# asharakeh/pod_compare

Hardware: AMD Instinct MI355X
Metric: images/sec (BayesOD+MC-dropout, 1280x720) (higher is better)
Workload: dtype f32 (convolutions: every fp32 product from 2-way f16 splits of the power-of-two-scaled fp32 operands, 3 partial products, fp32 accumulate; closer to fp64 than the fp32 MFMA: profiles/r05_f16_split_numerics.txt)

## Files before the change

### pod_compare_amd/csrc/k11_wino_conv.hip

```cpp
#include "pod_wino.h"

namespace pod {

__global__ void __launch_bounds__(256) k_wino_filter(const float* __restrict__ w, float* __restrict__ U, int32_t K, int32_t C, int32_t Kpad) {
    const int64_t t = (int64_t)blockIdx.x * blockDim.x + threadIdx.x;
    if (t >= (int64_t)Kpad * C) return;
    const int k = (int)(t / C), c = (int)(t % C);
    float u[4][6];
    wino_filter_values(w, k, c, K, C, u);
    const int nchunk = C / 8, ks = k >> 6, j64 = k & 63, ch = c >> 3, cc = c & 7;
    const int h = cc >> 2, sc = cc & 3;
    float* dst = U + ((int64_t)ks * nchunk + ch) * WINO_U_FLOATS + (h * 64 + j64) * 4 + sc;
#pragma unroll
    for (int q = 0; q < 24; ++q) dst[q * 512] = u[q / 6][q % 6];
}

__global__ void __launch_bounds__(256, 1) k_wino_conv3x3(const WinoParams P) {
    extern __shared__ __attribute__((aligned(16))) float lds[];
    const int tid = threadIdx.x, lane = tid & 63, wave = tid >> 6;
    int ks, tb;
    wino_schedule(P.KS, P.n_blocks, ks, tb);
    if (tb >= P.n_blocks) return;
    WINO_STAMP(0);
    WINO_STAMP_WALL(12);
// ... 125 lines not shown
    __builtin_amdgcn_s_waitcnt(WINO_WAIT_VM16);
    __builtin_amdgcn_s_barrier();
    WINO_STAMP(1);
    WINO_READ_MINI(0, 0); WINO_READ_MINI(0, 1); WINO_READ_MINI(0, 2); WINO_READ_MINI(0, 3); WINO_READ_MINI(0, 4); WINO_READ_MINI(0, 5);
    WINO_READ_MINI(0, 6); WINO_READ_MINI(0, 7); WINO_READ_MINI(0, 8); WINO_READ_MINI(0, 9); WINO_READ_MINI(0, 10); WINO_READ_MINI(0, 11);
    __builtin_amdgcn_s_waitcnt(WINO_WAIT_LGKM0);
    __builtin_amdgcn_sched_barrier(0);
#pragma unroll
    for (int i = 0; i < 10; ++i) transform_piece(vA, i);
    __builtin_amdgcn_sched_barrier(0);
    asm volatile("s_nop 1");
    WINO_STAMP(2);
    const f32x16 zero16 = {0.f, 0.f, 0.f, 0.f, 0.f, 0.f, 0.f, 0.f, 0.f, 0.f, 0.f, 0.f, 0.f, 0.f, 0.f, 0.f};
    auto chunk = [&](auto first, auto c_t, auto par_t, int sc, f32x4(&vC)[6], f32x4(&uC)[12], f32x4(&vN)[6], f32x4(&uN)[12]) {
        constexpr int c = decltype(c_t)::value, par = decltype(par_t)::value;
        constexpr int rc = (c + 1) & 3, rpar = c == 3 ? par ^ 1 : par;
        constexpr int ph = c == 3 ? 0 : c + 1, dpar = c == 3 ? par : par ^ 1;
        const int ch = 4 * sc + c, c1 = ch + 1 < nchunk ? ch + 1 : last;
        const int fs0 = c == 3 ? sc + 2 : sc + 1, fs = fs0 < last_s ? fs0 : last_s;
        float* wr = lds + dpar * WINO_SB_FLOATS;
        wino_static_for([&](auto J) __attribute__((always_inline)) {
            constexpr int j = decltype(J)::value;
            if constexpr (decltype(first)::value && j < 12) acc[j] = __builtin_amdgcn_mfma_f32_32x32x2f32(uC[j][0], vC[j >> 1][0], zero16, 0, 0, 0);
            else WINO_MFMA(vC, uC, j);
            if constexpr (j < 12) {
                if constexpr (decltype(first)::value) WINO_READ_MINI(1, j);
                else if (!(POD_WINO_ELIM & 1)) WINO_READ(rpar, rc, j);
            }
            else if constexpr (j < 24) { if (!(POD_WINO_ELIM & 2)) filter_piece(c1, uN, j - 12); }
            else if constexpr (j == 24) __builtin_amdgcn_s_waitcnt(WINO_WAIT_LGKM0);
            else if constexpr (j >= 25 && j < 35) { if (!(POD_WINO_ELIM & 8)) transform_piece(vN, j - 25); }
            else if constexpr (j >= 36 && j <= 45 && (j - 36) % 3 == 0 && c != 2) { if (!(POD_WINO_ELIM & 4)) wino_patch_piece(r_rsrc, wr, a, fs, 4 * ph + (j - 36) / 3, doff[4 * ph + (j - 36) / 3]); }
            __builtin_amdgcn_sched_barrier(0);
        }, std::make_integer_sequence<int, 48>{});
        if (!(POD_WINO_ELIM & 16)) {
            __builtin_amdgcn_s_waitcnt(c != 2 ? WINO_WAIT_VM4 : WINO_WAIT_VM0);
            __builtin_amdgcn_s_barrier();
        }
    };
    using std::integral_constant;
    chunk(std::true_type{}, integral_constant<int, 0>{}, integral_constant<int, 0>{}, 0, vA, uA, vB, uB);
    for (int base = 0;; base += 8) {
#define WINO_CHUNK(t)                                                                                                              \
    if (base + (t) >= nchunk) break;                                                                                               \
    if ((t) & 1) chunk(std::false_type{}, integral_constant<int, (t) & 3>{}, integral_constant<int, ((t) >> 2) & 1>{}, (base + (t)) >> 2, vB, uB, vA, uA); \
    else chunk(std::false_type{}, integral_constant<int, (t) & 3>{}, integral_constant<int, ((t) >> 2) & 1>{}, (base + (t)) >> 2, vA, uA, vB, uB);
        WINO_CHUNK(1) WINO_CHUNK(2) WINO_CHUNK(3) WINO_CHUNK(4) WINO_CHUNK(5) WINO_CHUNK(6) WINO_CHUNK(7) WINO_CHUNK(8)
#undef WINO_CHUNK
    }
#undef WINO_MFMA
    __syncthreads();
    WINO_STAMP(3);

    if (!wino_output_stage(acc, lds, a, i32, h)) return;
    const WinoStore S{P.sets.out[0], P.sets.bias[0], nullptr, 1.0f, P.sets.offset[0], 0, P.sets.k_planes[0]};
    if (S.k_planes > 0) wino_store_planes(P, B, S, lds, ks);
    else wino_store_channels_last(P, B, S, lds, ks);
    WINO_STAMP_END();
}

}

#ifdef POD_TRACE
extern "C" int pod_wino_trace_dump(long long* host, int32_t n_workgroups) { return pod::wino_trace_dump(host, n_workgroups); }
#endif

extern "C" int pod_wino_filter_transform(const float* weight, float* U, int32_t K, int32_t C, pod_stream_t stream) {
    if (!weight || !U || K < 1 || C < 8 || (C & 7) != 0) return POD_E_INVALID;
    const int32_t Kpad = (K + 63) / 64 * 64;
    const int64_t n = (int64_t)Kpad * C;
    hipLaunchKernelGGL(pod::k_wino_filter, dim3((unsigned)((n + 255) / 256)), dim3(256), 0, (hipStream_t)stream, weight, U, K, C, Kpad);
    POD_CHECK_LAUNCH();
    return POD_OK;
}

extern "C" int pod_wino_conv3x3(const float* in, float* out, const float* U, const float* bias, const int32_t* blocks, int32_t n_blocks,
                                int32_t C, int32_t K, int32_t k_planes, int32_t relu, float p, uint64_t seed, uint64_t offset,
                                const uint64_t* epoch, pod_stream_t stream) {
    if (!in || !out || in == out || !U || !blocks || n_blocks < 0 || C < 8 || (C & 7) != 0 || K < 64 || (K & 63) != 0 ||
        !(p >= 0.0f && p < 1.0f) || k_planes < 0 || k_planes > K || (k_planes > 0 && p != 0.0f))
        return POD_E_INVALID;
    pod::WinoParams P{};
    const int64_t grid = pod::wino_params_launch(P, blocks, n_blocks, C, K, relu, p, seed, epoch);
    if (grid < 0) return POD_E_INVALID;
    if (((reinterpret_cast<uintptr_t>(in) | reinterpret_cast<uintptr_t>(out) | reinterpret_cast<uintptr_t>(U) |
          reinterpret_cast<uintptr_t>(bias) | reinterpret_cast<uintptr_t>(blocks)) & 15u) != 0)
        return POD_E_INVALID;
    if (n_blocks == 0) return POD_OK;
    if (pod_lds_opt_in<pod::k_wino_conv3x3>(pod::WINO_LDS_BYTES) != POD_OK) return POD_E_LAUNCH;
    pod::wino_params_set(P, 0, 0, in, out, U, bias, nullptr, nullptr, offset, 0, k_planes);
    hipLaunchKernelGGL(pod::k_wino_conv3x3, dim3((unsigned)grid), dim3(256), pod::WINO_LDS_BYTES, (hipStream_t)stream, P);
    POD_CHECK_LAUNCH();
    return POD_OK;
}
```

### pod_compare_amd/csrc/k12_wino_conv_split.hip

```cpp
#include "pod_wino.h"

namespace pod {

typedef uint32_t vu32x4 __attribute__((ext_vector_type(4)));
constexpr int WINO_US_BYTES = 24 * 2 * 2 * 64 * 16;
constexpr int WINO_U_TOP = 14, WINO_V_TOP = 9;
constexpr int WINO_WAIT_VM24 = 0x4078;

__global__ void __launch_bounds__(256) k_wino_filter_amax(const float* __restrict__ w, float* __restrict__ amax, int32_t K, int32_t C, int32_t Kpad) {
    const int64_t t = (int64_t)blockIdx.x * blockDim.x + threadIdx.x;
    float m = 0.0f;
    if (t < (int64_t)Kpad * C) {
        float u[4][6];
        wino_filter_values(w, (int)(t / C), (int)(t % C), K, C, u);
#pragma unroll
        for (int i = 0; i < 24; ++i) m = fmaxf(m, fabsf(u[i / 6][i % 6]));
    }
    wino_publish_amax1(amax, m);
}
__global__ void __launch_bounds__(256) k_wino_filter_split(const float* __restrict__ w, uint16_t* __restrict__ Us, const float* __restrict__ amax,
                                                           int32_t K, int32_t C, int32_t Kpad) {
    const int64_t t = (int64_t)blockIdx.x * blockDim.x + threadIdx.x;
    if (t >= (int64_t)Kpad * C) return;
    const int k = (int)(t / C), c = (int)(t % C);
// ... 270 lines not shown
            if constexpr (mode == 0 && prod == 0)
                acc[p * 2 + kb] = __builtin_amdgcn_mfma_f32_32x32x16_f16(__builtin_bit_cast(wino_f16x8, uP[p][kb * 2 + sa]), __builtin_bit_cast(wino_f16x8, Vb[p][sb]), zero16, 0, 0, 0);
            else
                acc[p * 2 + kb] = __builtin_amdgcn_mfma_f32_32x32x16_f16(__builtin_bit_cast(wino_f16x8, uP[p][kb * 2 + sa]), __builtin_bit_cast(wino_f16x8, Vb[p][sb]), acc[p * 2 + kb], 0, 0, 0);
            if constexpr (m < 4) { if (!(POD_WINO_ELIM & 2)) filter_piece(p + WINO_U_LEAD >= 6 ? qn : q, (p + WINO_U_LEAD) % 6, uP[(p + WINO_U_LEAD) % 6], m); }
            else if constexpr (m == 4) { if (!(POD_WINO_ELIM & 4)) stage_write(c16 == 0 ? par ^ 1 : par, p, c16 == 0 ? 6 + p : p); }
            if constexpr (p == 5 && m >= 4) {
                if (!(POD_WINO_ELIM & 4)) {
                    stage_load(3 * (m - 4), ls, 6 * c16 + 3 * (m - 4));
                    stage_load(3 * (m - 4) + 1, ls, 6 * c16 + 3 * (m - 4) + 1);
                    stage_load(3 * (m - 4) + 2, ls, 6 * c16 + 3 * (m - 4) + 2);
                }
            }
            if constexpr (mode != 0) {
                constexpr int u0 = j * N_UNITS / N_SLOTS, u1 = (j + 1) * N_UNITS / N_SLOTS;
                wino_static_for([&](auto K) __attribute__((always_inline)) {
                    unit(std::integral_constant<int, u0 + decltype(K)::value>{}, std::integral_constant<int, npar>{}, std::integral_constant<int, n16>{},
                         std::integral_constant<bool, mode == 2>{});
                }, std::make_integer_sequence<int, u1 - u0>{});
            }
            __builtin_amdgcn_sched_barrier(0);
        }, std::make_integer_sequence<int, N_SLOTS>{});
        __builtin_amdgcn_s_waitcnt(WINO_WAIT_LGKM0);
        __builtin_amdgcn_s_barrier();
        if constexpr (mode == 0) {
            if (q >= last) return;
            if constexpr (!(POD_WINO_ELIM & 1)) WINO_READ12(WINO_READ, npar, n16, 0);
            WINO_READS_LANDED();
            __builtin_amdgcn_sched_barrier(0);
            make_v(0);
            __builtin_amdgcn_sched_barrier(0);
            if constexpr (!(POD_WINO_ELIM & 1)) WINO_READ12(WINO_READ, npar, n16, 1);
            WINO_READS_LANDED();
            __builtin_amdgcn_sched_barrier(0);
            make_v(1);
            split_all();
            __builtin_amdgcn_sched_barrier(0);
            __builtin_amdgcn_s_barrier();
        }
    };
    using std::integral_constant;
    chunk(integral_constant<int, 0>{}, integral_constant<int, 0>{}, integral_constant<int, 0>{}, 0);
    if (nchunk > 1) chunk(integral_constant<int, 1>{}, integral_constant<int, 1>{}, integral_constant<int, 0>{}, 1);
    for (int base = 0;; base += 4) {
#define WINO_CHUNK(t)                                                                                                              \
    if (base + (t) >= nchunk) break;                                                                                               \
    chunk(integral_constant<int, 2>{}, integral_constant<int, (t) & 1>{}, integral_constant<int, ((t) >> 1) & 1>{}, base + (t));
        WINO_CHUNK(2) WINO_CHUNK(3) WINO_CHUNK(4) WINO_CHUNK(5)
#undef WINO_CHUNK
    }
    __syncthreads();
    WINO_STAMP(3);

    if (!wino_output_stage(acc, lds, a, i32, h)) return;
    const float inv = wino_pow2_inverse(sv) * wino_pow2_inverse(wino_pow2_scale(u_amax, WINO_U_TOP));
    const WinoStore S{set_out + (int64_t)blockIdx.y * P.split_out_stride, set_bias, set_out_amax, inv, set_offset, set_replicas, set_k_planes};
    const float lmax = S.k_planes > 0 ? wino_store_planes(P, B, S, lds, ks) : wino_store_channels_last(P, B, S, lds, ks);
    if (set_out_amax) wino_publish_amax_block(set_out_amax, lmax);
    WINO_STAMP_END();
}

}

#ifdef POD_TRACE
extern "C" int pod_wino_trace_dump_split(long long* host, int32_t n_workgroups) { return pod::wino_trace_dump(host, n_workgroups); }
#endif

extern "C" int64_t pod_wino_filter_split_bytes(int32_t K, int32_t C) {
    if (K < 1 || C < 16 || (C & 15) != 0) return 0;
    const int64_t Kpad = (K + 63) / 64 * 64;
    return Kpad / 64 * (C / 16) * (int64_t)pod::WINO_US_BYTES + 16;
}

extern "C" int pod_wino_filter_transform_split(const float* weight, void* Us, int32_t K, int32_t C, pod_stream_t stream) {
    if (!weight || !Us || K < 1 || C < 16 || (C & 15) != 0 || (reinterpret_cast<uintptr_t>(Us) & 15u) != 0) return POD_E_INVALID;
    const int32_t Kpad = (K + 63) / 64 * 64;
    const int64_t n = (int64_t)Kpad * C;
    float* amax = reinterpret_cast<float*>(reinterpret_cast<char*>(Us) + pod_wino_filter_split_bytes(K, C) - 16);
    if (hipMemsetAsync(amax, 0, 16, (hipStream_t)stream) != hipSuccess) return POD_E_LAUNCH;
    hipLaunchKernelGGL(pod::k_wino_filter_amax, dim3((unsigned)((n + 255) / 256)), dim3(256), 0, (hipStream_t)stream, weight, amax, K, C, Kpad);
    POD_CHECK_LAUNCH();
    hipLaunchKernelGGL(pod::k_wino_filter_split, dim3((unsigned)((n + 255) / 256)), dim3(256), 0, (hipStream_t)stream, weight,
                       reinterpret_cast<uint16_t*>(Us), amax, K, C, Kpad);
    POD_CHECK_LAUNCH();
    return POD_OK;
}

extern "C" int pod_wino_conv3x3_split(const PodWinoConv* d, pod_stream_t stream) {
    if (!d || d->n_sets < 1 || d->n_sets > 4 || !d->blocks || d->n_blocks < 0 || d->C < 16 || (d->C & 15) != 0 || d->K < 64 || (d->K & 63) != 0 ||
        !(d->p >= 0.0f && d->p < 1.0f) || d->sets[0].first_block != 0 || (reinterpret_cast<uintptr_t>(d->blocks) & 15u) != 0 ||
        d->reserved != 0)
        return POD_E_INVALID;
    const int32_t C = d->C, K = d->K;
    pod::WinoParams P{};
    const int64_t grid = pod::wino_params_launch(P, d->blocks, d->n_blocks, C, K, d->relu, d->p, d->seed, d->epoch);
    if (grid < 0) return POD_E_INVALID;
    const bool partial = d->n_splits > 1;
    if (partial) {
        if (d->n_sets != 1 || d->n_splits > 16 || (C / 16) % d->n_splits != 0 || ((C / 16 / d->n_splits) & 1) != 0 || d->split_stride < 0 || (d->split_stride & 3) != 0 ||
            d->p != 0.0f || d->relu || d->sets[0].bias || d->sets[0].replicas || d->sets[0].k_planes || d->sets[0].out_amax)
            return POD_E_INVALID;
    }
    for (int s = 0; s < 4; ++s) {
        const PodConvSet& q = d->sets[s < d->n_sets ? s : 0];
        if (s < d->n_sets) {
            if (!q.in || !q.out || q.in == q.out || !q.Us || !q.in_amax || q.replicas < 0 || q.replicas > 127 || q.k_planes < 0 || q.k_planes > K ||
                (q.k_planes > 0 && (d->p != 0.0f || q.replicas != 0)) || (s > 0 && q.first_block < d->sets[s - 1].first_block) || q.first_block > d->n_blocks)
                return POD_E_INVALID;
            if (((reinterpret_cast<uintptr_t>(q.in) | reinterpret_cast<uintptr_t>(q.out) | reinterpret_cast<uintptr_t>(q.Us) | reinterpret_cast<uintptr_t>(q.bias)) & 15u) != 0 ||
                ((reinterpret_cast<uintptr_t>(q.in_amax) | reinterpret_cast<uintptr_t>(q.out_amax)) & 3u) != 0)
// ... 13 lines not shown
```

### pod_compare_amd/csrc/pod_device.h

```cpp
#pragma once

#include <hip/hip_runtime.h>
#include <stdint.h>

#include <mutex>

#include "../../include/pod_mi355x.h"

#define POD_WAVE 64
#define POD_EPS_MAX 4.9f

#define POD_CHECK_LAUNCH()                                  \
    do {                                                    \
        if (hipGetLastError() != hipSuccess) return POD_E_LAUNCH; \
    } while (0)

template <auto Kernel>
static int pod_lds_opt_in(int bytes) {
    static std::once_flag once[64];
    static hipError_t attr[64];
    int dev = 0;
    if (hipGetDevice(&dev) != hipSuccess || dev < 0 || dev >= 64) return POD_E_LAUNCH;
    std::call_once(once[dev], [dev, bytes] {
        attr[dev] = hipFuncSetAttribute(reinterpret_cast<const void*>(Kernel), hipFuncAttributeMaxDynamicSharedMemorySize, bytes);
    });
    return attr[dev] == hipSuccess ? POD_OK : POD_E_LAUNCH;
}

#ifdef POD_TRACE
static __device__ long long g_pod_trace[4096 * 8];
#define POD_STAMP(wg, k)                                                                         \
    do {                                                                                         \
        if ((threadIdx.x & 63) == 0 && threadIdx.x < 64 && (wg) < 4096) g_pod_trace[(wg) * 8 + (k)] = wall_clock64(); \
    } while (0)
#else
#define POD_STAMP(wg, k)
#endif

namespace pod {

struct u32x4 {
    uint32_t x, y, z, w;
};

__device__ __forceinline__ u32x4 philox4x32_10(u32x4 c, uint32_t k0, uint32_t k1) {
    constexpr uint32_t M0 = 0xD2511F53u, M1 = 0xCD9E8D57u, W0 = 0x9E3779B9u, W1 = 0xBB67AE85u;
#pragma unroll
    for (int r = 0; r < 10; ++r) {
        const uint64_t p0 = (uint64_t)M0 * c.x;
        const uint64_t p1 = (uint64_t)M1 * c.z;
        u32x4 n;
        n.x = (uint32_t)(p1 >> 32) ^ c.y ^ k0;
        n.y = (uint32_t)p1;
        n.z = (uint32_t)(p0 >> 32) ^ c.w ^ k1;
        n.w = (uint32_t)p0;
        c = n;
        k0 += W0;
        k1 += W1;
    }
    return c;
}

__device__ __forceinline__ uint64_t dropout_key(uint64_t seed, const uint64_t* epoch) {
    return epoch ? seed ^ (*epoch * 0x9E3779B97F4A7C15ull) : seed;
}

__device__ __forceinline__ void dropout_words(uint64_t base, uint64_t g, uint32_t c2, uint32_t stream, uint64_t seed, uint32_t& w0, uint32_t& w1) {
    const uint64_t ctr = base + (g >> 1);
    const u32x4 r = philox4x32_10(u32x4{(uint32_t)ctr, (uint32_t)(ctr >> 32), c2, stream}, (uint32_t)seed, (uint32_t)(seed >> 32));
    w0 = (g & 1) ? r.z : r.x;
    w1 = (g & 1) ? r.w : r.y;
}
#define POD_DROPOUT_THRESH16(p) ((uint32_t)((double)(p) * 65536.0))

__device__ __forceinline__ void box_muller16(uint32_t w, float& n0, float& n1) {
    const float u1 = ((float)(w & 0xFFFFu) + 0.5f) * 1.52587890625e-05f;
    const float u2 = ((float)(w >> 16) + 0.5f) * 1.52587890625e-05f;
    const float rad = __builtin_amdgcn_sqrtf(-1.3862943611198906f * __builtin_amdgcn_logf(u1));
    n0 = rad * __builtin_amdgcn_cosf(u2);
    n1 = rad * __builtin_amdgcn_sinf(u2);
}

struct f32x8n {
    float v[8];
};

constexpr uint32_t STREAM_CLS = 0x636c7300u;
constexpr uint32_t STREAM_BOX = 0x626f7800u;

__device__ __forceinline__ f32x8n philox_normals8(uint64_t seed, uint32_t c0, uint32_t c1, uint32_t c2, uint32_t stream) {
    const u32x4 r = philox4x32_10(u32x4{c0, c1, c2, stream}, (uint32_t)seed, (uint32_t)(seed >> 32));
    f32x8n o;
    box_muller16(r.x, o.v[0], o.v[1]);
    box_muller16(r.y, o.v[2], o.v[3]);
    box_muller16(r.z, o.v[4], o.v[5]);
    box_muller16(r.w, o.v[6], o.v[7]);
    return o;
}


__device__ __forceinline__ float sigmoid_ref(float x) { return __fdiv_rn(1.0f, 1.0f + expf(-x)); }
__device__ __forceinline__ float sigmoid_fast(float x) {
    return __builtin_amdgcn_rcpf(1.0f + __builtin_amdgcn_exp2f(-1.4426950408889634f * x));
}

struct Box {
    float x1, y1, x2, y2;
// ... 72 lines not shown
```

### pod_compare_amd/csrc/pod_wino.h

```cpp
#pragma once
#include "pod_experiments.h"
#include "pod_split_gemm.h"

namespace pod {

constexpr uint32_t STREAM_DROPOUT_CONV = 0x64726f70u;

constexpr int WINO_U_FLOATS = 24 * 2 * 64 * 4;
constexpr int WINO_SB_FLOATS = 384 * 32;
constexpr int WINO_LDS_BYTES = 4 * 32 * 4 * 65 * 4;

#ifdef POD_TRACE
static __device__ long long g_wino_trace[8192 * 16];
#define WINO_STAMP(k)                                                                                          \
    do {                                                                                                       \
        if (threadIdx.x == 0 && blockIdx.x < 8192) g_wino_trace[blockIdx.x * 16 + (k)] = __builtin_readcyclecounter(); \
    } while (0)
#define WINO_STAMP_WALL(k)                                                                                     \
    do {                                                                                                       \
        if (threadIdx.x == 0 && blockIdx.x < 8192) g_wino_trace[blockIdx.x * 16 + (k)] = wall_clock64();       \
    } while (0)
#define WINO_STAMP_END()                                                                                       \
    do {                                                                                                       \
        __builtin_amdgcn_s_waitcnt(0);                                                                         \
        WINO_STAMP(5);                                                                                         \
        WINO_STAMP_WALL(13);                                                                                   \
        if (threadIdx.x == 0 && blockIdx.x < 8192) {                                                           \
            uint32_t hw, xcc;                                                                                  \
            asm volatile("s_getreg_b32 %0, hwreg(HW_REG_HW_ID)" : "=s"(hw));                                   \
            asm volatile("s_getreg_b32 %0, hwreg(HW_REG_XCC_ID)" : "=s"(xcc));                                 \
            g_wino_trace[blockIdx.x * 16 + 6] = ((long long)xcc << 32) | hw;                                   \
        }                                                                                                      \
    } while (0)
static inline int wino_trace_dump(long long* host, int32_t n_workgroups) {
    if (hipDeviceSynchronize() != hipSuccess) return POD_E_LAUNCH;
    if (n_workgroups > 8192) n_workgroups = 8192;
    if (hipMemcpyFromSymbol(host, HIP_SYMBOL(g_wino_trace), (size_t)n_workgroups * 16 * sizeof(long long)) != hipSuccess) return POD_E_LAUNCH;
    return POD_OK;
}
#else
#define WINO_STAMP(k)
#define WINO_STAMP_WALL(k)
#define WINO_STAMP_END()
#endif

constexpr int WINO_WAIT_VM4 = 0x0074, WINO_WAIT_VM0 = 0x0070, WINO_WAIT_VM16 = 0x4070, WINO_WAIT_LGKM0 = 0xC07F;

struct WinoParams {
    const int4* blocks;
    int32_t n_blocks, C, K, KS, in_stride, out_stride, relu;
    uint32_t thresh;
    float scale;
    uint64_t seed;
    int32_t c_split;
    int64_t split_out_stride;
    const uint64_t* epoch;
    const int32_t* live;
    struct Sets {
        int32_t first[4];
        const float* in[4];
        float* out[4];
        const float* U[4];
        const float* bias[4];
        const float* in_amax[4];
        float* out_amax[4];
        uint64_t offset[4];
        int32_t replicas[4];
        int32_t k_planes[4];
    } sets;
};

struct WinoSlotTable {
    uint32_t v[384];
    constexpr WinoSlotTable() : v() {
        for (int p = 0; p < 384; ++p) {
            const int cls = p & 1, k = p >> 1, rr = k / 18, px = k - rr * 18;
            const int py = cls ? (rr < 4 ? rr + 4 : rr + 8) : (rr < 4 ? rr : rr < 8 ? rr + 4 : rr + 8);
            const bool ok = cls ? rr < 8 : rr < 10;
            v[p] = ok ? (uint32_t)((py * 18 + px) | ((((px >> 2) & 3) + 4 * ((py >> 1) & 1)) << 16)) : 324u;
        }
    }
};
static __device__ const WinoSlotTable g_wino_slots{};

__device__ __forceinline__ void wino_schedule(int KS, int n_blocks, int& ks, int& tb) {
    const int xcd = blockIdx.x & 7, wi = (int)(blockIdx.x >> 3);
    const int SP = KS >= 2 ? 2 : 1, G = KS / SP;
    ks = SP * (xcd % G) + (wi % SP);
    tb = (wi / SP) * (8 / G) + xcd / G;
}
inline int64_t wino_grid(int KS, int64_t n_blocks) {
    const int SP = KS >= 2 ? 2 : 1, G = KS / SP;
    return 8 * SP * ((n_blocks * G + 7) / 8);
}
inline int64_t wino_params_launch(WinoParams& P, const int32_t* blocks, int32_t n_blocks, int32_t C, int32_t K, int32_t relu, float p, uint64_t seed,
                                  const uint64_t* epoch) {
// ... 91 lines not shown

#define WINO_FILL_SLOTS(slot_e, mini_pidx, tid)                                                                                       \
    _Pragma("unroll") for (int i = 0; i < 12; ++i) (slot_e)[i] = g_wino_slots.v[96 * ((tid) >> 6) + 8 * i + (((tid) & 63) >> 3)];     \
    _Pragma("unroll") for (int r = 0; r < 3; ++r) {                                                                                   \
        const int pp = ((((tid) >> 6) * 3 + r) * 64 + ((tid) & 63)) >> 1, py = pp / 21, pi = pp - py * 21, px = 4 * (pi % 5) + pi / 5; \
        (mini_pidx)[r] = py < 18 && pi < 20 && px < 18 ? py * 18 + px : 324;                                                          \
    }
__device__ __forceinline__ int wino_byte_offset(const WinoParams* P, int pix, int part4) {
    return pix >= 0 ? (pix * P->in_stride + part4) * 4 : 0x7FFFFF00;
}
__device__ __forceinline__ void wino_mini_offsets(const WinoParams* P, const int* pix_tab, const int (&mini_pidx)[3], int (&dmini)[3], int lane) {
#pragma unroll
    for (int r = 0; r < 3; ++r) dmini[r] = pix_tab[mini_pidx[r]];
#pragma unroll
    for (int r = 0; r < 3; ++r) dmini[r] = wino_byte_offset(P, dmini[r], 4 * (lane & 1));
}
typedef __attribute__((address_space(3))) void wino_lds_void;
__device__ __forceinline__ void wino_mini_piece(__amdgpu_buffer_rsrc_t rsrc, float* lds, int a, int which, int r, int dmini_r) {
    __builtin_amdgcn_raw_ptr_buffer_load_lds(rsrc, (wino_lds_void*)(lds + 2 * WINO_SB_FLOATS + which * 3072 + (a * 3 + r) * 256), 16, dmini_r, which * 32, 0, 0);
}
__device__ __forceinline__ void wino_patch_piece(__amdgpu_buffer_rsrc_t rsrc, float* stage, int a, int sc, int i, int doff_i) {
    __builtin_amdgcn_raw_ptr_buffer_load_lds(rsrc, (wino_lds_void*)(stage + (a * 12 + i) * 256), 16, doff_i, sc * 128, 0, 0);
}

constexpr int WINO_TS = 260;
constexpr int WINO_ZA = 32 * WINO_TS;
__device__ __forceinline__ bool wino_output_stage(const f32x16 (&acc)[12], float* lds, int a, int i32, int h) {
    if (POD_WINO_ELIM & 128) {
#pragma unroll
        for (int i = 0; i < 12; ++i) asm volatile("" ::"v"(acc[i]));
        return false;
    }
#pragma unroll
    for (int kb = 0; kb < 2; ++kb)
#pragma unroll
        for (int g = 0; g < 4; ++g) {
            f32x4 m[6];
#pragma unroll
            for (int p6 = 0; p6 < 6; ++p6) m[p6] = f32x4{acc[p6 * 2 + kb][4 * g], acc[p6 * 2 + kb][4 * g + 1], acc[p6 * 2 + kb][4 * g + 2], acc[p6 * 2 + kb][4 * g + 3]};
            const f32x4 s1 = m[1] + m[2], d1 = m[1] - m[2], s2 = m[3] + m[4], d2 = m[3] - m[4];
            float* o = lds + (a * 32 + i32) * WINO_TS + kb * 32 + 8 * g + 4 * h;
            *reinterpret_cast<f32x4*>(o) = (m[0] + s1) + s2;
            *reinterpret_cast<f32x4*>(o + 64) = __builtin_elementwise_fma(f32x4{2.f, 2.f, 2.f, 2.f}, d2, d1);
            *reinterpret_cast<f32x4*>(o + 128) = __builtin_elementwise_fma(f32x4{4.f, 4.f, 4.f, 4.f}, s2, s1);
            *reinterpret_cast<f32x4*>(o + 192) = __builtin_elementwise_fma(f32x4{8.f, 8.f, 8.f, 8.f}, d2, d1) + m[5];
        }
    __syncthreads();
    WINO_STAMP(4);
    return !(POD_WINO_ELIM & 32);
}

struct WinoStore {
    float* out;
    const float* bias;
    float* out_amax;
    float inv;
    uint64_t offset;
    int replicas, k_planes;
};
__device__ __forceinline__ void wino_dropout8(f32x4& v0, f32x4& v1, int64_t e, uint64_t offset, uint32_t word, uint64_t key, uint32_t thresh, float scale) {
    const uint64_t ctr = offset + (uint64_t)(e >> 3);
    const u32x4 r4 = philox4x32_10(u32x4{(uint32_t)ctr, (uint32_t)(ctr >> 32), word, STREAM_DROPOUT_CONV}, (uint32_t)key, (uint32_t)(key >> 32));
    v0.x = (r4.x & 0xFFFFu) >= thresh ? v0.x * scale : 0.f;
    v0.y = (r4.x >> 16) >= thresh ? v0.y * scale : 0.f;
    v0.z = (r4.y & 0xFFFFu) >= thresh ? v0.z * scale : 0.f;
    v0.w = (r4.y >> 16) >= thresh ? v0.w * scale : 0.f;
    v1.x = (r4.z & 0xFFFFu) >= thresh ? v1.x * scale : 0.f;
    v1.y = (r4.z >> 16) >= thresh ? v1.y * scale : 0.f;
    v1.z = (r4.w & 0xFFFFu) >= thresh ? v1.z * scale : 0.f;
    v1.w = (r4.w >> 16) >= thresh ? v1.w * scale : 0.f;
}

__device__ __forceinline__ float wino_store_planes(const WinoParams& P, const WinoBlock& B, const WinoStore& S, const float* lds, int ks) {
    const int tid = threadIdx.x;
    float lmax = 0.0f;
    const f32x4 inv = f32x4{S.inv, S.inv, S.inv, S.inv};
    const int oy = (tid >> 2) & 15, ox = (tid & 3) * 4;
    int m;
    const int gy = wino_cell(B.y0 + oy, B.Hv, B.rHv, m);
    int64_t px0[4];
#pragma unroll
    for (int e = 0; e < 4; ++e) {
        int n;
        const int gx = wino_cell(B.x0 + ox + e, B.Wv, B.rWv, n), img = m * B.gcols + n;
        px0[e] = (n < B.gcols && img < B.n_img && gx < B.W && gy < B.H) ? (B.out_px + (int64_t)img * B.HWi) * S.k_planes + (int64_t)gy * B.W + gx : -1;
    }
    const bool vec = px0[0] >= 0 && px0[3] == px0[0] + 3 && (px0[0] & 3) == 0 && (B.HWi & 3) == 0;
    const int tile = (oy >> 1) * 4 + (tid & 3);
#pragma unroll 2
    for (int it = 0; it < 16; ++it) {
        const int k = it * 4 + (tid >> 6), kg = ks * 64 + k;
        if (kg >= S.k_planes) continue;
        const float bias = S.bias ? S.bias[kg] : 0.0f;
        float y[4];
#pragma unroll
        for (int e = 0; e < 4; ++e) {
            const float* r = lds + tile * WINO_TS + e * 64 + k;
            y[e] = (oy & 1) == 0 ? (r[0] + r[WINO_ZA]) + r[2 * WINO_ZA] : (r[WINO_ZA] - r[2 * WINO_ZA]) - r[3 * WINO_ZA];
        }
        f32x4 v = __builtin_elementwise_fma(f32x4{y[0], y[1], y[2], y[3]}, inv, f32x4{bias, bias, bias, bias});
        if (P.relu) wino_relu4(v);
        if (S.out_amax)
            lmax = wino_absmax4(lmax, f32x4{px0[0] >= 0 ? v.x : 0.f, px0[1] >= 0 ? v.y : 0.f, px0[2] >= 0 ? v.z : 0.f, px0[3] >= 0 ? v.w : 0.f});
        float* plane = S.out + (int64_t)kg * B.HWi;
        if (vec) {
            *reinterpret_cast<f32x4*>(plane + px0[0]) = v;
        } else {
            if (px0[0] >= 0) plane[px0[0]] = v.x;
            if (px0[1] >= 0) plane[px0[1]] = v.y;
            if (px0[2] >= 0) plane[px0[2]] = v.z;
            if (px0[3] >= 0) plane[px0[3]] = v.w;
        }
    }
    return lmax;
}

__device__ __forceinline__ float wino_store_channels_last(const WinoParams& P, const WinoBlock& B, const WinoStore& S, const float* lds, int ks) {
    const int tid = threadIdx.x;
    float lmax = 0.0f;
    const f32x4 inv = f32x4{S.inv, S.inv, S.inv, S.inv};
    const int k8 = (tid & 7) * 8, kg = ks * 64 + k8, ox = (tid >> 3) & 15, odd = tid >> 7;
    f32x4 bias0 = f32x4{0.f, 0.f, 0.f, 0.f}, bias1 = bias0;
    if (S.bias) {
        bias0 = *reinterpret_cast<const f32x4*>(S.bias + kg);
        bias1 = *reinterpret_cast<const f32x4*>(S.bias + kg + 4);
    }
    const uint64_t drop_key = P.thresh ? dropout_key(P.seed, P.epoch) : 0ull;
    int n;
    const int gx = wino_cell(B.x0 + ox, B.Wv, B.rWv, n);
    const bool col_ok = n < B.gcols && gx < B.W;
    int m, gy = wino_cell(B.y0 + odd, B.Hv, B.rHv, m) - 2;
    const float* rbase = lds + (ox >> 2) * WINO_TS + (ox & 3) * 64 + k8 + (odd ? WINO_ZA : 0);
#pragma unroll 1
    for (int g = 0; g < 2; ++g) {
        f32x4 z[4][6];
        int gyi[4], imgi[4];
#pragma unroll
        for (int it = 0; it < 4; ++it) {
            gy += 2;
            if (gy >= B.Hv) {
                gy -= B.Hv;
                ++m;
            }
            gyi[it] = gy;
            imgi[it] = m * B.gcols + n;
            const float* r = rbase + (4 * g + it) * 4 * WINO_TS;
            z[it][0] = *reinterpret_cast<const f32x4*>(r); z[it][1] = *reinterpret_cast<const f32x4*>(r + 4);
            z[it][2] = *reinterpret_cast<const f32x4*>(r + WINO_ZA); z[it][3] = *reinterpret_cast<const f32x4*>(r + WINO_ZA + 4);
            z[it][4] = *reinterpret_cast<const f32x4*>(r + 2 * WINO_ZA); z[it][5] = *reinterpret_cast<const f32x4*>(r + 2 * WINO_ZA + 4);
        }
#pragma unroll
        for (int it = 0; it < 4; ++it) {
            const int gy_ = gyi[it], img = imgi[it];
            if (!col_ok || gy_ >= B.H || img >= B.n_img) continue;
            f32x4 v0 = __builtin_elementwise_fma(odd ? (z[it][0] - z[it][2]) - z[it][4] : (z[it][0] + z[it][2]) + z[it][4], inv, bias0);
            f32x4 v1 = __builtin_elementwise_fma(odd ? (z[it][1] - z[it][3]) - z[it][5] : (z[it][1] + z[it][3]) + z[it][5], inv, bias1);
            if (P.relu) {
                wino_relu4(v0);
                wino_relu4(v1);
            }
            int64_t e = (B.out_px + (int64_t)img * B.HWi + (int64_t)gy_ * B.W + gx) * P.out_stride + kg;
            if (S.out_amax) {
                const f32x4 a0v = __builtin_elementwise_abs(v0), a1v = __builtin_elementwise_abs(v1);
                const float mx = fmaxf(fmaxf(fmaxf(a0v.x, a0v.y), fmaxf(a0v.z, a0v.w)), fmaxf(fmaxf(a1v.x, a1v.y), fmaxf(a1v.z, a1v.w)));
                lmax = fmaxf(lmax, P.thresh ? mx * P.scale : mx);
            }
            if (S.replicas > 0) {
                for (int rep = 0; rep < S.replicas; ++rep, e += (int64_t)B.HWi * P.out_stride) {
                    f32x4 w0 = v0, w1 = v1;
                    if (P.thresh) wino_dropout8(w0, w1, e, S.offset, 2u, drop_key, P.thresh, P.scale);
                    *reinterpret_cast<f32x4*>(S.out + e) = w0;
                    *reinterpret_cast<f32x4*>(S.out + e + 4) = w1;
                }
                continue;
            }
            if (P.thresh && !(POD_WINO_ELIM & 64)) wino_dropout8(v0, v1, e, S.offset, 0u, drop_key, P.thresh, P.scale);
            *reinterpret_cast<f32x4*>(S.out + e) = v0;
            *reinterpret_cast<f32x4*>(S.out + e + 4) = v1;
        }
    }
    return lmax;
}

}
```

Measured before the change: 131.4.

## Hoist Winograd epilogue bias/epoch loads before output stage and streamline plane store

Bias and dropout-epoch global loads are issued before the output-transform stage, so their latency overlaps the LDS transform instead of stalling the store epilogue. In the planes path, each lane loads one bias value up front and it is broadcast with readlane instead of a per-iteration scalar load. The row combine is rewritten as sign-select FMAs over a fixed LDS base. Philox XORs use a three-input bitop instruction, and cycle-lap trace macros are added for debug builds only. The hoisted values add register pressure that persists across the output stage.

```diff
diff --git a/pod_compare_amd/csrc/k11_wino_conv.hip b/pod_compare_amd/csrc/k11_wino_conv.hip
--- a/pod_compare_amd/csrc/k11_wino_conv.hip
+++ b/pod_compare_amd/csrc/k11_wino_conv.hip
@@ -201,10 +201,11 @@
     __syncthreads();
     WINO_STAMP(3);
 
+    const WinoStoreLoads L = wino_store_loads(P, P.sets.bias[0], P.sets.k_planes[0], ks);
     if (!wino_output_stage(acc, lds, a, i32, h)) return;
-    const WinoStore S{P.sets.out[0], P.sets.bias[0], nullptr, 1.0f, P.sets.offset[0], 0, P.sets.k_planes[0]};
-    if (S.k_planes > 0) wino_store_planes(P, B, S, lds, ks);
-    else wino_store_channels_last(P, B, S, lds, ks);
+    const WinoStore S{P.sets.out[0], nullptr, 1.0f, P.sets.offset[0], 0, P.sets.k_planes[0]};
+    if (S.k_planes > 0) wino_store_planes(P, B, S, L, lds, ks);
+    else wino_store_channels_last(P, B, S, L, lds, ks);
     WINO_STAMP_END();
 }
 
diff --git a/pod_compare_amd/csrc/k12_wino_conv_split.hip b/pod_compare_amd/csrc/k12_wino_conv_split.hip
--- a/pod_compare_amd/csrc/k12_wino_conv_split.hip
+++ b/pod_compare_amd/csrc/k12_wino_conv_split.hip
@@ -346,10 +346,11 @@
     __syncthreads();
     WINO_STAMP(3);
 
+    const WinoStoreLoads L = wino_store_loads(P, set_bias, set_k_planes, ks);
     if (!wino_output_stage(acc, lds, a, i32, h)) return;
     const float inv = wino_pow2_inverse(sv) * wino_pow2_inverse(wino_pow2_scale(u_amax, WINO_U_TOP));
-    const WinoStore S{set_out + (int64_t)blockIdx.y * P.split_out_stride, set_bias, set_out_amax, inv, set_offset, set_replicas, set_k_planes};
-    const float lmax = S.k_planes > 0 ? wino_store_planes(P, B, S, lds, ks) : wino_store_channels_last(P, B, S, lds, ks);
+    const WinoStore S{set_out + (int64_t)blockIdx.y * P.split_out_stride, set_out_amax, inv, set_offset, set_replicas, set_k_planes};
+    const float lmax = S.k_planes > 0 ? wino_store_planes(P, B, S, L, lds, ks) : wino_store_channels_last(P, B, S, L, lds, ks);
     if (set_out_amax) wino_publish_amax_block(set_out_amax, lmax);
     WINO_STAMP_END();
 }
diff --git a/pod_compare_amd/csrc/pod_device.h b/pod_compare_amd/csrc/pod_device.h
--- a/pod_compare_amd/csrc/pod_device.h
+++ b/pod_compare_amd/csrc/pod_device.h
@@ -43,6 +43,14 @@
     uint32_t x, y, z, w;
 };
 
+__device__ __forceinline__ uint32_t xor3(uint32_t a, uint32_t b, uint32_t c) {
+#if defined(__HIP_DEVICE_COMPILE__) && __has_builtin(__builtin_amdgcn_bitop3_b32)
+    return __builtin_amdgcn_bitop3_b32(a, b, c, 0x96);
+#else
+    return a ^ b ^ c;
+#endif
+}
+
 __device__ __forceinline__ u32x4 philox4x32_10(u32x4 c, uint32_t k0, uint32_t k1) {
     constexpr uint32_t M0 = 0xD2511F53u, M1 = 0xCD9E8D57u, W0 = 0x9E3779B9u, W1 = 0xBB67AE85u;
 #pragma unroll
@@ -50,9 +58,9 @@
         const uint64_t p0 = (uint64_t)M0 * c.x;
         const uint64_t p1 = (uint64_t)M1 * c.z;
         u32x4 n;
-        n.x = (uint32_t)(p1 >> 32) ^ c.y ^ k0;
+        n.x = xor3((uint32_t)(p1 >> 32), c.y, k0);
         n.y = (uint32_t)p1;
-        n.z = (uint32_t)(p0 >> 32) ^ c.w ^ k1;
+        n.z = xor3((uint32_t)(p0 >> 32), c.w, k1);
         n.w = (uint32_t)p0;
         c = n;
         k0 += W0;
diff --git a/pod_compare_amd/csrc/pod_wino.h b/pod_compare_amd/csrc/pod_wino.h
--- a/pod_compare_amd/csrc/pod_wino.h
+++ b/pod_compare_amd/csrc/pod_wino.h
@@ -38,10 +38,28 @@
     if (hipMemcpyFromSymbol(host, HIP_SYMBOL(g_wino_trace), (size_t)n_workgroups * 16 * sizeof(long long)) != hipSuccess) return POD_E_LAUNCH;
     return POD_OK;
 }
+#define WINO_LAPS_BEGIN() long long lap_mark_ = __builtin_readcyclecounter(), lap_sum_[2] = {0, 0}
+#define WINO_LAP(i, ...)                                                                                       \
+    do {                                                                                                       \
+        wino_pin(__VA_ARGS__);                                                                                 \
+        const long long now_ = __builtin_readcyclecounter();                                                   \
+        lap_sum_[i] += now_ - lap_mark_;                                                                       \
+        lap_mark_ = now_;                                                                                      \
+    } while (0)
+#define WINO_LAPS_END(k)                                                                                       \
+    do {                                                                                                       \
+        if (threadIdx.x == 0 && blockIdx.x < 8192) {                                                           \
+            g_wino_trace[blockIdx.x * 16 + (k)] = lap_sum_[0];                                                 \
+            g_wino_trace[blockIdx.x * 16 + (k) + 1] = lap_sum_[1];                                             \
+        }                                                                                                      \
+    } while (0)
 #else
 #define WINO_STAMP(k)
 #define WINO_STAMP_WALL(k)
 #define WINO_STAMP_END()
+#define WINO_LAPS_BEGIN()
+#define WINO_LAP(i, ...)
+#define WINO_LAPS_END(k)
 #endif
 
 constexpr int WINO_WAIT_VM4 = 0x0074, WINO_WAIT_VM0 = 0x0070, WINO_WAIT_VM16 = 0x4070, WINO_WAIT_LGKM0 = 0xC07F;
@@ -239,12 +257,43 @@
 
 struct WinoStore {
     float* out;
-    const float* bias;
     float* out_amax;
     float inv;
     uint64_t offset;
     int replicas, k_planes;
 };
+struct WinoStoreLoads {
+    f32x4 bias0, bias1;
+    float bias_lane;
+    uint32_t epoch[2];
+};
+__device__ __forceinline__ WinoStoreLoads wino_store_loads(const WinoParams& P, const float* bias, int k_planes, int ks) {
+    const int tid = threadIdx.x;
+    WinoStoreLoads L;
+    if (k_planes > 0) {
+        const int kg = ks * 64 + (tid & 63);
+        L.bias_lane = bias ? bias[kg < k_planes ? kg : k_planes - 1] : 0.0f;
+        return L;
+    }
+    const int kg = ks * 64 + (tid & 7) * 8;
+    L.bias0 = bias ? *reinterpret_cast<const f32x4*>(bias + kg) : f32x4{0.f, 0.f, 0.f, 0.f};
+    L.bias1 = bias ? *reinterpret_cast<const f32x4*>(bias + kg + 4) : f32x4{0.f, 0.f, 0.f, 0.f};
+    if (P.thresh && P.epoch) {
+        const uint64_t w = *P.epoch;
+        L.epoch[0] = (uint32_t)w;
+        L.epoch[1] = (uint32_t)(w >> 32);
+    }
+    return L;
+}
+__device__ __forceinline__ uint64_t wino_store_key(const WinoParams& P, const WinoStoreLoads& L) {
+    if (!P.thresh) return 0ull;
+    if (!P.epoch) return P.seed;
+    uint32_t lo = L.epoch[0], hi = L.epoch[1];
+    wino_pin(lo, hi);
+    const uint64_t w = ((uint64_t)hi << 32) | lo;
+    return dropout_key(P.seed, &w);
+}
+
 __device__ __forceinline__ void wino_dropout8(f32x4& v0, f32x4& v1, int64_t e, uint64_t offset, uint32_t word, uint64_t key, uint32_t thresh, float scale) {
     const uint64_t ctr = offset + (uint64_t)(e >> 3);
     const u32x4 r4 = philox4x32_10(u32x4{(uint32_t)ctr, (uint32_t)(ctr >> 32), word, STREAM_DROPOUT_CONV}, (uint32_t)key, (uint32_t)(key >> 32));
@@ -258,8 +307,8 @@
     v1.w = (r4.w >> 16) >= thresh ? v1.w * scale : 0.f;
 }
 
-__device__ __forceinline__ float wino_store_planes(const WinoParams& P, const WinoBlock& B, const WinoStore& S, const float* lds, int ks) {
-    const int tid = threadIdx.x;
+__device__ __forceinline__ float wino_store_planes(const WinoParams& P, const WinoBlock& B, const WinoStore& S, const WinoStoreLoads& L, const float* lds, int ks) {
+    const int tid = threadIdx.x, wave = __builtin_amdgcn_readfirstlane(tid >> 6);
     float lmax = 0.0f;
     const f32x4 inv = f32x4{S.inv, S.inv, S.inv, S.inv};
     const int oy = (tid >> 2) & 15, ox = (tid & 3) * 4;
@@ -273,18 +322,29 @@
         px0[e] = (n < B.gcols && img < B.n_img && gx < B.W && gy < B.H) ? (B.out_px + (int64_t)img * B.HWi) * S.k_planes + (int64_t)gy * B.W + gx : -1;
     }
     const bool vec = px0[0] >= 0 && px0[3] == px0[0] + 3 && (px0[0] & 3) == 0 && (B.HWi & 3) == 0;
-    const int tile = (oy >> 1) * 4 + (tid & 3);
+    const bool odd = (oy & 1) != 0;
+    const float* const zbase = lds + ((oy >> 1) * 4 + (tid & 3)) * WINO_TS + (odd ? WINO_ZA : 0);
+    const float sgn = odd ? -1.0f : 1.0f;
+    int bias_lanes = __builtin_bit_cast(int, L.bias_lane);
+#ifdef POD_TRACE
+    wino_pin(bias_lanes, px0[0], px0[1], px0[2], px0[3]);
+#endif
+    WINO_STAMP(7);
+    WINO_LAPS_BEGIN();
 #pragma unroll 2
     for (int it = 0; it < 16; ++it) {
-        const int k = it * 4 + (tid >> 6), kg = ks * 64 + k;
+        const int k = it * 4 + wave, kg = ks * 64 + k;
         if (kg >= S.k_planes) continue;
-        const float bias = S.bias ? S.bias[kg] : 0.0f;
+        const float bias = __builtin_bit_cast(float, __builtin_amdgcn_readlane(bias_lanes, k));
+        float z[4][3];
+#pragma unroll
+        for (int e = 0; e < 4; ++e)
+#pragma unroll
+            for (int j = 0; j < 3; ++j) z[e][j] = zbase[j * WINO_ZA + e * 64 + k];
+        WINO_LAP(0, z[0][0], z[0][1], z[0][2], z[1][0], z[1][1], z[1][2], z[2][0], z[2][1], z[2][2], z[3][0], z[3][1], z[3][2]);
         float y[4];
 #pragma unroll
-        for (int e = 0; e < 4; ++e) {
-            const float* r = lds + tile * WINO_TS + e * 64 + k;
-            y[e] = (oy & 1) == 0 ? (r[0] + r[WINO_ZA]) + r[2 * WINO_ZA] : (r[WINO_ZA] - r[2 * WINO_ZA]) - r[3 * WINO_ZA];
-        }
+        for (int e = 0; e < 4; ++e) y[e] = __builtin_fmaf(sgn, z[e][2], __builtin_fmaf(sgn, z[e][1], z[e][0]));
         f32x4 v = __builtin_elementwise_fma(f32x4{y[0], y[1], y[2], y[3]}, inv, f32x4{bias, bias, bias, bias});
         if (P.relu) wino_relu4(v);
         if (S.out_amax)
@@ -298,21 +358,19 @@
             if (px0[2] >= 0) plane[px0[2]] = v.z;
             if (px0[3] >= 0) plane[px0[3]] = v.w;
         }
-    }
+        WINO_LAP(1, v);
+    }
+    WINO_LAPS_END(14);
     return lmax;
 }
 
-__device__ __forceinline__ float wino_store_channels_last(const WinoParams& P, const WinoBlock& B, const WinoStore& S, const float* lds, int ks) {
+__device__ __forceinline__ float wino_store_channels_last(const WinoParams& P, const WinoBlock& B, const WinoStore& S, const WinoStoreLoads& L, const float* lds, int ks) {
     const int tid = threadIdx.x;
     float lmax = 0.0f;
     const f32x4 inv = f32x4{S.inv, S.inv, S.inv, S.inv};
     const int k8 = (tid & 7) * 8, kg = ks * 64 + k8, ox = (tid >> 3) & 15, odd = tid >> 7;
-    f32x4 bias0 = f32x4{0.f, 0.f, 0.f, 0.f}, bias1 = bias0;
-    if (S.bias) {
-        bias0 = *reinterpret_cast<const f32x4*>(S.bias + kg);
-        bias1 = *reinterpret_cast<const f32x4*>(S.bias + kg + 4);
-    }
-    const uint64_t drop_key = P.thresh ? dropout_key(P.seed, P.epoch) : 0ull;
+    const f32x4 bias0 = L.bias0, bias1 = L.bias1;
+    const uint64_t drop_key = wino_store_key(P, L);
     int n;
     const int gx = wino_cell(B.x0 + ox, B.Wv, B.rWv, n);
     const bool col_ok = n < B.gcols && gx < B.W;
```

Measured after the change: 132.2 (median of 2 runs). About the same (+0.6%).

## Specialize Winograd output stores on relu/amax/dropout and batch per-wave store loops

Applied to the files above, without the earlier changes.

Turns the plane and channels-last Winograd output-store routines into templates specialized on relu, amax and dropout, so those branches are resolved at compile time. The plane store now batches four k-planes per iteration, with bias read once per lane and broadcast through readlane. Output addresses are advanced incrementally instead of recomputed, and the odd/even row selection becomes a signed FMA. Replica writes are restructured to loop over replicas outside the row group. The intent is to cut scalar/vector ALU work, branching and address arithmetic in the epilogue, at the cost of more code and higher register pressure from the batched loads.

```diff
diff --git a/pod_compare_amd/csrc/pod_wino.h b/pod_compare_amd/csrc/pod_wino.h
--- a/pod_compare_amd/csrc/pod_wino.h
+++ b/pod_compare_amd/csrc/pod_wino.h
@@ -258,11 +258,17 @@
     v1.w = (r4.w >> 16) >= thresh ? v1.w * scale : 0.f;
 }
 
-__device__ __forceinline__ float wino_store_planes(const WinoParams& P, const WinoBlock& B, const WinoStore& S, const float* lds, int ks) {
-    const int tid = threadIdx.x;
+
+template <bool RELU, bool AMAX>
+__device__ __forceinline__ float wino_store_planes_form(const WinoBlock& B, const WinoStore& S, const float* lds, int ks) {
+    const int tid = threadIdx.x, wave = __builtin_amdgcn_readfirstlane(tid >> 6);
     float lmax = 0.0f;
     const f32x4 inv = f32x4{S.inv, S.inv, S.inv, S.inv};
-    const int oy = (tid >> 2) & 15, ox = (tid & 3) * 4;
+    const int oy = (tid >> 2) & 15, ox = (tid & 3) * 4, odd = oy & 1;
+    const float sg = odd ? -1.0f : 1.0f;
+    const int kg0 = ks * 64 + wave;
+    const int n_it = (S.k_planes - kg0 + 3) >> 2;
+    const float bias_l = S.bias ? S.bias[kg0 + 4 * (tid & 15)] : 0.0f;
     int m;
     const int gy = wino_cell(B.y0 + oy, B.Hv, B.rHv, m);
     int64_t px0[4];
@@ -273,64 +279,102 @@
         px0[e] = (n < B.gcols && img < B.n_img && gx < B.W && gy < B.H) ? (B.out_px + (int64_t)img * B.HWi) * S.k_planes + (int64_t)gy * B.W + gx : -1;
     }
     const bool vec = px0[0] >= 0 && px0[3] == px0[0] + 3 && (px0[0] & 3) == 0 && (B.HWi & 3) == 0;
+    const bool ok[4] = {px0[0] >= 0, px0[1] >= 0, px0[2] >= 0, px0[3] >= 0};
+    int64_t q[4];
+#pragma unroll
+    for (int e = 0; e < 4; ++e) q[e] = (int64_t)kg0 * B.HWi + px0[e];
+    const int64_t q_it = (int64_t)4 * B.HWi;
     const int tile = (oy >> 1) * 4 + (tid & 3);
-#pragma unroll 2
-    for (int it = 0; it < 16; ++it) {
-        const int k = it * 4 + (tid >> 6), kg = ks * 64 + k;
-        if (kg >= S.k_planes) continue;
-        const float bias = S.bias ? S.bias[kg] : 0.0f;
-        float y[4];
-#pragma unroll
-        for (int e = 0; e < 4; ++e) {
-            const float* r = lds + tile * WINO_TS + e * 64 + k;
-            y[e] = (oy & 1) == 0 ? (r[0] + r[WINO_ZA]) + r[2 * WINO_ZA] : (r[WINO_ZA] - r[2 * WINO_ZA]) - r[3 * WINO_ZA];
-        }
-        f32x4 v = __builtin_elementwise_fma(f32x4{y[0], y[1], y[2], y[3]}, inv, f32x4{bias, bias, bias, bias});
-        if (P.relu) wino_relu4(v);
-        if (S.out_amax)
-            lmax = wino_absmax4(lmax, f32x4{px0[0] >= 0 ? v.x : 0.f, px0[1] >= 0 ? v.y : 0.f, px0[2] >= 0 ? v.z : 0.f, px0[3] >= 0 ? v.w : 0.f});
-        float* plane = S.out + (int64_t)kg * B.HWi;
-        if (vec) {
-            *reinterpret_cast<f32x4*>(plane + px0[0]) = v;
-        } else {
-            if (px0[0] >= 0) plane[px0[0]] = v.x;
-            if (px0[1] >= 0) plane[px0[1]] = v.y;
-            if (px0[2] >= 0) plane[px0[2]] = v.z;
-            if (px0[3] >= 0) plane[px0[3]] = v.w;
+    const float* r = lds + tile * WINO_TS + wave + (odd ? WINO_ZA : 0);
+#pragma unroll 1
+    for (int it0 = 0; it0 < 16 && it0 < n_it; it0 += 4, r += 16) {
+        float z[4][4][3];
+        f32x4 v[4];
+#pragma unroll
+        for (int j = 0; j < 4; ++j)
+#pragma unroll
+            for (int e = 0; e < 4; ++e)
+#pragma unroll
+                for (int a = 0; a < 3; ++a) z[j][e][a] = r[4 * j + e * 64 + a * WINO_ZA];
+#pragma unroll
+        for (int j = 0; j < 4; ++j) {
+            const float bias = __builtin_bit_cast(float, __builtin_amdgcn_readlane(__builtin_bit_cast(int, bias_l), it0 + j));
+            f32x4 y;
+#pragma unroll
+            for (int e = 0; e < 4; ++e) y[e] = __builtin_fmaf(sg, z[j][e][2], __builtin_fmaf(sg, z[j][e][1], z[j][e][0]));
+            v[j] = __builtin_elementwise_fma(y, inv, f32x4{bias, bias, bias, bias});
+            if (RELU) wino_relu4(v[j]);
+            if (AMAX) {
+                const float mx = wino_absmax4(0.0f, f32x4{ok[0] ? v[j].x : 0.f, ok[1] ? v[j].y : 0.f, ok[2] ? v[j].z : 0.f, ok[3] ? v[j].w : 0.f});
+                lmax = fmaxf(lmax, it0 + j < n_it ? mx : 0.0f);
+            }
+        }
+        wino_pin(v[0], v[1], v[2], v[3]);
+#pragma unroll
+        for (int j = 0; j < 4; ++j) {
+            const bool live = it0 + j < n_it;
+            if (live && vec) {
+                *reinterpret_cast<f32x4*>(S.out + q[0]) = v[j];
+            } else if (live) {
+                if (ok[0]) S.out[q[0]] = v[j].x;
+                if (ok[1]) S.out[q[1]] = v[j].y;
+                if (ok[2]) S.out[q[2]] = v[j].z;
+                if (ok[3]) S.out[q[3]] = v[j].w;
+            }
+#pragma unroll
+            for (int e = 0; e < 4; ++e) q[e] += q_it;
         }
     }
     return lmax;
 }
-
-__device__ __forceinline__ float wino_store_channels_last(const WinoParams& P, const WinoBlock& B, const WinoStore& S, const float* lds, int ks) {
+__device__ __forceinline__ float wino_store_planes(const WinoParams& P, const WinoBlock& B, const WinoStore& S, const float* lds, int ks) {
+    switch ((P.relu ? 1 : 0) | (S.out_amax ? 2 : 0)) {
+        case 0: return wino_store_planes_form<false, false>(B, S, lds, ks);
+        case 1: return wino_store_planes_form<true, false>(B, S, lds, ks);
+        case 2: return wino_store_planes_form<false, true>(B, S, lds, ks);
+        default: return wino_store_planes_form<true, true>(B, S, lds, ks);
+    }
+}
+
+template <bool RELU, bool DROP>
+__device__ __forceinline__ float wino_store_channels_last_form(const WinoParams& P, const WinoBlock& B, const WinoStore& S, const float* lds, int ks) {
     const int tid = threadIdx.x;
     float lmax = 0.0f;
     const f32x4 inv = f32x4{S.inv, S.inv, S.inv, S.inv};
     const int k8 = (tid & 7) * 8, kg = ks * 64 + k8, ox = (tid >> 3) & 15, odd = tid >> 7;
+    const float sg1 = odd ? -1.0f : 1.0f;
+    const f32x4 sg = f32x4{sg1, sg1, sg1, sg1};
     f32x4 bias0 = f32x4{0.f, 0.f, 0.f, 0.f}, bias1 = bias0;
     if (S.bias) {
         bias0 = *reinterpret_cast<const f32x4*>(S.bias + kg);
         bias1 = *reinterpret_cast<const f32x4*>(S.bias + kg + 4);
     }
-    const uint64_t drop_key = P.thresh ? dropout_key(P.seed, P.epoch) : 0ull;
-    int n;
+    const uint64_t drop_key = DROP ? dropout_key(P.seed, P.epoch) : 0ull;
+    const int n_rep = S.replicas > 0 ? S.replicas : 1;
+    const uint32_t word = S.replicas > 0 ? 2u : 0u;
+    int n, m;
     const int gx = wino_cell(B.x0 + ox, B.Wv, B.rWv, n);
     const bool col_ok = n < B.gcols && gx < B.W;
-    int m, gy = wino_cell(B.y0 + odd, B.Hv, B.rHv, m) - 2;
+    int gy = wino_cell(B.y0 + odd, B.Hv, B.rHv, m);
+    int img = m * B.gcols + n;
+    const int64_t e_row = (int64_t)(2 * B.W) * P.out_stride, e_wrap = ((int64_t)B.gcols * B.HWi - (int64_t)B.Hv * B.W) * P.out_stride, e_rep = (int64_t)B.HWi * P.out_stride;
+    int64_t e = (B.out_px + (int64_t)img * B.HWi + (int64_t)gy * B.W + gx) * P.out_stride + kg - e_row;
+    gy -= 2;
     const float* rbase = lds + (ox >> 2) * WINO_TS + (ox & 3) * 64 + k8 + (odd ? WINO_ZA : 0);
 #pragma unroll 1
     for (int g = 0; g < 2; ++g) {
-        f32x4 z[4][6];
-        int gyi[4], imgi[4];
+        f32x4 z[4][6], v[4][2];
+        bool ok[4];
+        int64_t er[4];
 #pragma unroll
         for (int it = 0; it < 4; ++it) {
             gy += 2;
-            if (gy >= B.Hv) {
-                gy -= B.Hv;
-                ++m;
-            }
-            gyi[it] = gy;
-            imgi[it] = m * B.gcols + n;
+            const bool wrap = gy >= B.Hv;
+            gy -= wrap ? B.Hv : 0;
+            img += wrap ? B.gcols : 0;
+            e += e_row + (wrap ? e_wrap : 0);
+            ok[it] = col_ok && gy < B.H && img < B.n_img;
+            er[it] = e;
             const float* r = rbase + (4 * g + it) * 4 * WINO_TS;
             z[it][0] = *reinterpret_cast<const f32x4*>(r); z[it][1] = *reinterpret_cast<const f32x4*>(r + 4);
             z[it][2] = *reinterpret_cast<const f32x4*>(r + WINO_ZA); z[it][3] = *reinterpret_cast<const f32x4*>(r + WINO_ZA + 4);
@@ -338,35 +382,45 @@
         }
 #pragma unroll
         for (int it = 0; it < 4; ++it) {
-            const int gy_ = gyi[it], img = imgi[it];
-            if (!col_ok || gy_ >= B.H || img >= B.n_img) continue;
-            f32x4 v0 = __builtin_elementwise_fma(odd ? (z[it][0] - z[it][2]) - z[it][4] : (z[it][0] + z[it][2]) + z[it][4], inv, bias0);
-            f32x4 v1 = __builtin_elementwise_fma(odd ? (z[it][1] - z[it][3]) - z[it][5] : (z[it][1] + z[it][3]) + z[it][5], inv, bias1);
-            if (P.relu) {
-                wino_relu4(v0);
-                wino_relu4(v1);
+            v[it][0] = __builtin_elementwise_fma(__builtin_elementwise_fma(sg, z[it][4], __builtin_elementwise_fma(sg, z[it][2], z[it][0])), inv, bias0);
+            v[it][1] = __builtin_elementwise_fma(__builtin_elementwise_fma(sg, z[it][5], __builtin_elementwise_fma(sg, z[it][3], z[it][1])), inv, bias1);
+            if (RELU) {
+                wino_relu4(v[it][0]);
+                wino_relu4(v[it][1]);
             }
-            int64_t e = (B.out_px + (int64_t)img * B.HWi + (int64_t)gy_ * B.W + gx) * P.out_stride + kg;
-            if (S.out_amax) {
-                const f32x4 a0v = __builtin_elementwise_abs(v0), a1v = __builtin_elementwise_abs(v1);
-                const float mx = fmaxf(fmaxf(fmaxf(a0v.x, a0v.y), fmaxf(a0v.z, a0v.w)), fmaxf(fmaxf(a1v.x, a1v.y), fmaxf(a1v.z, a1v.w)));
-                lmax = fmaxf(lmax, P.thresh ? mx * P.scale : mx);
+            const float mx = wino_absmax4(wino_absmax4(0.0f, v[it][0]), v[it][1]);
+            lmax = fmaxf(lmax, ok[it] ? (DROP ? mx * P.scale : mx) : 0.0f);
+        }
+#pragma unroll 1
+        for (int rep = 0; rep < n_rep; ++rep) {
+            f32x4 w[4][2];
+#pragma unroll
+            for (int it = 0; it < 4; ++it) {
+                w[it][0] = v[it][0];
+                w[it][1] = v[it][1];
+                if (DROP && !(POD_WINO_ELIM & 64)) wino_dropout8(w[it][0], w[it][1], er[it], S.offset, word, drop_key, P.thresh, P.scale);
             }
-            if (S.replicas > 0) {
-                for (int rep = 0; rep < S.replicas; ++rep, e += (int64_t)B.HWi * P.out_stride) {
-                    f32x4 w0 = v0, w1 = v1;
-                    if (P.thresh) wino_dropout8(w0, w1, e, S.offset, 2u, drop_key, P.thresh, P.scale);
-                    *reinterpret_cast<f32x4*>(S.out + e) = w0;
-                    *reinterpret_cast<f32x4*>(S.out + e + 4) = w1;
+#pragma unroll
+            for (int it = 0; it < 4; ++it) wino_pin(w[it][0], w[it][1]);
+#pragma unroll
+            for (int it = 0; it < 4; ++it) {
+                if (ok[it]) {
+                    *reinterpret_cast<f32x4*>(S.out + er[it]) = w[it][0];
+                    *reinterpret_cast<f32x4*>(S.out + er[it] + 4) = w[it][1];
                 }
-                continue;
+                er[it] += e_rep;
             }
-            if (P.thresh && !(POD_WINO_ELIM & 64)) wino_dropout8(v0, v1, e, S.offset, 0u, drop_key, P.thresh, P.scale);
-            *reinterpret_cast<f32x4*>(S.out + e) = v0;
-            *reinterpret_cast<f32x4*>(S.out + e + 4) = v1;
         }
     }
     return lmax;
 }
-
-}
+__device__ __forceinline__ float wino_store_channels_last(const WinoParams& P, const WinoBlock& B, const WinoStore& S, const float* lds, int ks) {
+    switch ((P.relu ? 1 : 0) | (P.thresh ? 2 : 0)) {
+        case 0: return wino_store_channels_last_form<false, false>(P, B, S, lds, ks);
+        case 1: return wino_store_channels_last_form<true, false>(P, B, S, lds, ks);
+        case 2: return wino_store_channels_last_form<false, true>(P, B, S, lds, ks);
+        default: return wino_store_channels_last_form<true, true>(P, B, S, lds, ks);
+    }
+}
+
+}
```

Result: faster. 139.1 before, 142.3 after, median of 6 (+2.3%).
